# anihcsam/OpenGaussian

Measured on AMD Instinct MI355X. Metric: fwd+bwd Mpix/s at 1080p, 1M Gaussians (RGB+6-D ins_feat); k-means it/s, higher is better.
Workload: dtype f32; 1 GPU; S1M-1080p RGB(SH3)+depth+alpha (all grads) + 6-ch ins_feat (grad to ins_feat) fwd+bwd, ONE fused 9-channel pass; gaussians=1000000, width=1920, height=1080, views_cycled=8, parallelism=single

## Files before the change

opengaussian_amd/csrc/capi.hip:

```cpp
#include <stdarg.h>
#include <stdlib.h>
#include <string.h>

#include <map>
#include <mutex>
#include <string>
#include <vector>

#include "ogs_common.h"

namespace ogs {

static thread_local char g_err[512] = "";

void set_error(const char* fmt, ...) {
    va_list ap;
    va_start(ap, fmt);
    vsnprintf(g_err, sizeof(g_err), fmt, ap);
    va_end(ap);
}

namespace {
struct ProfRec { const char* name; hipEvent_t start, stop; };
int g_prof_mode = 0;
// ... 40 lines not shown
        memset(p, 0, 64);
        g_async_status = static_cast<uint32_t*>(p);
    }
    return g_async_status;
}
int take_async_status() {
    std::lock_guard<std::mutex> lk(g_async_mu);
    if (!g_async_status) return 0;
    return (int)__atomic_exchange_n(g_async_status, 0u, __ATOMIC_ACQ_REL);
}
int check_async_status(const char* where) {
    const int st = take_async_status();
    if (st == 0) return OGS_OK;
    set_error("%s: a kernel of an earlier launch reported status 0x%x%s -- the results of the passes since the last check "
              "are not valid", where, st,
              (st & (int)kAsyncRadixSpin) ? " (one-launch radix pass: a look-back wait exceeded its bound)" : "");
    return OGS_ERR_DEVICE;
}

}
int ogs::blend_prefetch_lines() {
    static const int v = [] {
        const char* e = getenv("OGS_BLEND_PREFETCH");
        const int n = e ? atoi(e) : kPrefetchMax;
        const int lines = (n & 0xFF) > kPrefetchMax ? kPrefetchMax : (n & 0xFF);
#ifdef OGS_EXPERIMENTS
        return n < 0 ? 0 : (lines | (n & 0x300));
#else
        return n < 0 ? 0 : lines;
#endif
    }();
    return v;
}
namespace ogs {

static int bit_length(uint32_t v) {
    int n = 0;
    while (v) { ++n; v >>= 1; }
    return n;
}

static int validate_fwd(const OgsRasterFwdArgs* a, bool images = true) {
    if (!a) { set_error("args == NULL"); return OGS_ERR_INVALID_ARG; }
    if (a->P < 0 || a->W <= 0 || a->H <= 0) { set_error("bad sizes P=%d W=%d H=%d", a->P, a->W, a->H); return OGS_ERR_INVALID_ARG; }
    if (a->C != 3 && a->C != 6 && a->C != 9 && a->C != 12) { set_error("C=%d unsupported (3, 6, 9, 12)", a->C); return OGS_ERR_UNSUPPORTED; }
    if (a->shs == nullptr && a->colors_precomp == nullptr) {
        set_error("provide shs or colors_precomp"); return OGS_ERR_INVALID_ARG;
    }
    if (a->shs != nullptr && (a->colors_precomp != nullptr) != (a->C > 3)) {
        set_error("with shs: C == 3 and no colors_precomp, or C > 3 with colors_precomp holding the C-3 extra channels");
        return OGS_ERR_INVALID_ARG;
    }
    const bool sr = a->scales != nullptr && a->rotations != nullptr;
    if (sr == (a->cov3D_precomp != nullptr) || (a->scales != nullptr) != (a->rotations != nullptr)) {
        set_error("provide exactly one of (scales, rotations) / cov3D_precomp"); return OGS_ERR_INVALID_ARG;
    }
    if (a->shs) {
        if (a->sh_degree < 0 || a->sh_degree > 3 || a->sh_coeffs < (a->sh_degree + 1) * (a->sh_degree + 1)) {
            set_error("sh_degree=%d needs >= %d coefficients, got %d", a->sh_degree, (a->sh_degree + 1) * (a->sh_degree + 1), a->sh_coeffs);
            return OGS_ERR_INVALID_ARG;
        }
    }
    if (!a->bg || !a->viewmatrix || !a->projmatrix || !a->campos || (images && (!a->out_color || !a->out_depth || !a->out_alpha))) {
        set_error("NULL required pointer"); return OGS_ERR_INVALID_ARG;
    }
    if (a->P > 0 && (!a->means3D || !a->opacities || !a->radii || !a->geom_buffer || !a->geom_tmp)) {
        set_error("NULL required per-Gaussian pointer"); return OGS_ERR_INVALID_ARG;
    }
    if (a->num_groups < 0 || (a->num_groups > 1 && a->P > 0 && !a->group_ids)) {
        set_error("num_groups=%d needs group_ids", a->num_groups); return OGS_ERR_INVALID_ARG;
    }
    return OGS_OK;
}

}

using namespace ogs;

extern "C" {

int ogs_version(void) { return 401; }

int ogs_check_async_status(void) { return check_async_status("ogs_check_async_status"); }

int ogs_prof_enable(int on) {
    std::lock_guard<std::mutex> lk(g_prof_mu);
    for (auto& r : g_prof) { g_event_pool.push_back(r.start); g_event_pool.push_back(r.stop); }
    g_prof.clear();
    g_prof_mode = on;
    return OGS_OK;
}

int ogs_prof_filter(const char* prefix) {
    std::lock_guard<std::mutex> lk(g_prof_mu);
    if (!prefix || strlen(prefix) >= sizeof(g_prof_prefix)) { set_error("prof_filter: prefix NULL or longer than %zu", sizeof(g_prof_prefix) - 1); return OGS_ERR_INVALID_ARG; }
    strcpy(g_prof_prefix, prefix);
    return OGS_OK;
}

int ogs_prof_collect(char* buf, size_t n) {
    std::lock_guard<std::mutex> lk(g_prof_mu);
    std::map<std::string, std::pair<long, double>> agg;
    for (auto& r : g_prof) {
        OGS_HIP_CHECK(hipEventSynchronize(r.stop));
        float ms = 0.f;
        OGS_HIP_CHECK(hipEventElapsedTime(&ms, r.start, r.stop));
        auto& a = agg[r.name];
        a.first += 1;
        a.second += ms;
    }
    std::string out = "{";
    bool first = true;
    for (auto& kv : agg) {
        char line[384];
// ... 8 lines not shown
    if (!buf || out.size() + 1 > n) { set_error("prof_collect: buffer too small (%zu needed)", out.size() + 1); return OGS_ERR_SCRATCH_TOO_SMALL; }
    memcpy(buf, out.c_str(), out.size() + 1);
    return OGS_OK;
}
const char* ogs_last_error(void) { return g_err; }

size_t ogs_raster_geom_bytes(int32_t P, int32_t C) { return GeomState::bytes(P > 0 ? P : 1, C); }
size_t ogs_raster_geom_tmp_bytes(int32_t P) { return GeomTmp::bytes(P > 0 ? P : 1); }
size_t ogs_raster_image_bytes(int32_t W, int32_t H) { return ImageState::bytes(W, H); }
size_t ogs_raster_image_bytes_grouped(int32_t W, int32_t H, int32_t G) { return ImageState::bytes(W, H, num_groups_of(G)); }
size_t ogs_raster_binning_tmp_bytes(int64_t D, int32_t, int32_t) { return BinTmp::bytes(D > 0 ? D : 1); }
size_t ogs_raster_sorted_bytes(int64_t D, int32_t C) {
    return align_up((size_t)(D > 0 ? D : 1) * stream_vec4(C) * sizeof(float4));
}
size_t ogs_raster_quad_list_bytes(int64_t D) {
    return align_up((size_t)(5 * (D > 0 ? D : 1) + 2 * kQuadPad) * sizeof(uint32_t));
}
size_t ogs_raster_backward_tmp_bytes(int32_t P) { return align_up((size_t)(P > 0 ? P : 1) * 16 * sizeof(double)); }

int ogs_raster_forward_geometry(const OgsRasterFwdArgs* a, void* stream_, int64_t* num_rendered_host) {
    int rc = validate_fwd(a, false);
    if (rc != OGS_OK) return rc;
    hipStream_t s = static_cast<hipStream_t>(stream_);
    if (num_rendered_host) *num_rendered_host = 0;
    if (a->P == 0) return OGS_OK;
    rc = check_async_status("forward (entry)");
    if (rc != OGS_OK) return rc;
    const GeomState gs = GeomState::carve(a->geom_buffer, a->P, a->C);
    const GeomTmp gt = GeomTmp::carve(a->geom_tmp, a->P);
    if (a->P <= kSmallMaxP) {
        rc = launch_small_geometry(*a, gs, gt, s);
        if (rc != OGS_OK) return rc;
    } else if (per_tile_depth_order(*a)) {
        rc = launch_preprocess(*a, gs, gt, s);
        if (rc != OGS_OK) return rc;
        rc = exclusive_scan_u32(gt.tiles_touched, nullptr, gt.offsets, a->P, gt.num_rendered, gt.sort_tmp, s, a->debug);
        if (rc != OGS_OK) return rc;
    } else {
        rc = launch_preprocess(*a, gs, gt, s);
        if (rc != OGS_OK) return rc;
        const bool sweep = radix_onesweep_enabled(a->P);
        if (sweep) {
            const int shifts[4] = {0, 8, 16, 24}, nbits[4] = {8, 8, 8, 8};
            rc = radix_sort_begin(gt.keys[0], a->P, nullptr, 4, shifts, nbits, gt.sort_tmp, s, a->debug, true);
            if (rc != OGS_OK) return rc;
        }
        for (int pass = 0; pass < 4; ++pass) {
            const int in = pass & 1, out = in ^ 1;
            const bool drop = pass == 0;
            const uint32_t* n_pass = drop ? nullptr : gt.visible();
            rc = sweep ? radix_sort_pass(pass, 4, gt.keys[in], gt.order[in], gt.keys[out], gt.order[out], a->P, 8 * pass, 8, gt.sort_tmp, s, a->debug, n_pass, drop, drop ? gt.visible() : nullptr)
                       : radix_pass(gt.keys[in], gt.order[in], gt.keys[out], gt.order[out], a->P, 8 * pass, 8, gt.sort_tmp, s, a->debug, n_pass, drop, drop ? gt.visible() : nullptr);
            if (rc != OGS_OK) return rc;
        }
        rc = exclusive_scan_u32(gt.tiles_touched, gt.order[0], gt.offsets, a->P, gt.num_rendered, gt.sort_tmp, s, a->debug, gt.visible());
        if (rc != OGS_OK) return rc;
    }
    if (num_rendered_host) {
        uint32_t d = 0;
        OGS_HIP_CHECK(hipMemcpyAsync(&d, gt.num_rendered, sizeof(uint32_t), hipMemcpyDeviceToHost, s));
        OGS_HIP_CHECK(hipStreamSynchronize(s));
        *num_rendered_host = (int64_t)d;
        rc = check_async_status("forward geometry phase");
        if (rc != OGS_OK) return rc;
    }
    return OGS_OK;
}

int ogs_raster_read_num_rendered_async(const OgsRasterFwdArgs* a, void* stream_, uint32_t* host_pinned) {
    if (!a || !host_pinned) { set_error("read_num_rendered_async: NULL pointer"); return OGS_ERR_INVALID_ARG; }
    if (a->P == 0) { *host_pinned = 0; return OGS_OK; }
    const GeomTmp gt = GeomTmp::carve(a->geom_tmp, a->P);
    OGS_HIP_CHECK(hipMemcpyAsync(host_pinned, gt.num_rendered, sizeof(uint32_t), hipMemcpyDeviceToHost,
                                 static_cast<hipStream_t>(stream_)));
    return OGS_OK;
}

static int render_impl(const OgsRasterFwdArgs* a, int64_t D, bool deferred, hipStream_t s,
                       const OgsGroupStatsArgs* stats = nullptr) {
    int rc = validate_fwd(a, stats == nullptr);
    if (rc != OGS_OK) return rc;
    if (!a->image_buffer) { set_error("image_buffer == NULL"); return OGS_ERR_INVALID_ARG; }
    const int G = num_groups_of(a->num_groups);
    const ImageState is = stats ? ImageState::carve_stats(a->image_buffer, a->W, a->H, G)
                                : ImageState::carve(a->image_buffer, a->W, a->H, G);
    const int gx = (a->W + kTile - 1) / kTile, gy = (a->H + kTile - 1) / kTile;
    const int64_t tiles = (int64_t)gx * gy * G;
    if (tiles >= (1ll << 31)) { set_error("%d groups x %d tiles exceed 2^31 virtual tiles", G, gx * gy); return OGS_ERR_UNSUPPORTED; }
    const GeomState gs = GeomState::carve(a->geom_buffer, a->P > 0 ? a->P : 1, a->C);
    const bool per_tile = per_tile_depth_order(*a);
    bool order_ready = false;
    if (D > 0) {
        if (!a->point_list || !a->binning_tmp) { set_error("point_list / binning_tmp == NULL with num_rendered=%lld", (long long)D); return OGS_ERR_INVALID_ARG; }
        if (D >= (1ll << 31)) { set_error("num_rendered=%lld exceeds 2^31", (long long)D); return OGS_ERR_UNSUPPORTED; }
        const GeomTmp gt = GeomTmp::carve(a->geom_tmp, a->P);
        const BinTmp bt = BinTmp::carve(a->binning_tmp, D);
        const int bits = bit_length((uint32_t)(tiles - 1));
        const int passes = bits == 0 ? 1 : (bits + 7) / 8;
        const int per = bits == 0 ? 1 : (bits + passes - 1) / passes;
        uint32_t* vbuf[2];
        vbuf[passes & 1] = a->point_list;
        vbuf[(passes & 1) ^ 1] = bt.vals;
        const uint32_t* n_dev = deferred ? gt.num_rendered : nullptr;
        const bool cull = a->full_binning == 0;
        const bool zero_in_dup = tiles <= (int64_t)a->P;
        rc = launch_duplicate(*a, gs, gt, bt.tile_keys[0], vbuf[0], (uint32_t)D, cull, !per_tile, s,
                              zero_in_dup ? is.ranges : nullptr, zero_in_dup ? (int)tiles : 0);
        if (rc != OGS_OK) return rc;
        const bool sweep = radix_onesweep_enabled(D);
        int shifts[4], nbits[4];
        for (int p = 0; p < passes; ++p) {
            shifts[p] = p * per;
            nbits[p] = (p == passes - 1) ? (bits == 0 ? 1 : bits - shifts[p]) : per;
        }
        if (passes == 2 && (bits & 1)) {
            nbits[0] = bits / 2; shifts[1] = nbits[0]; nbits[1] = bits - nbits[0];
        }
        if (sweep) {
            rc = radix_sort_begin(bt.tile_keys[0], D, n_dev, passes, shifts, nbits, bt.sort_tmp, s, a->debug, cull);
            if (rc != OGS_OK) return rc;
        }
        for (int p = 0; p < passes; ++p) {
            const int in = p & 1, out = in ^ 1;
            const bool drop = cull && p == 0;
            const uint32_t* n_pass = (cull && p > 0) ? bt.kept : n_dev;
            rc = sweep ? radix_sort_pass(p, passes, bt.tile_keys[in], vbuf[in], bt.tile_keys[out], vbuf[out], D, shifts[p], nbits[p], bt.sort_tmp, s, a->debug, n_pass, drop, drop ? bt.kept : nullptr)
                       : radix_pass(bt.tile_keys[in], vbuf[in], bt.tile_keys[out], vbuf[out], D, shifts[p], nbits[p], bt.sort_tmp, s, a->debug, n_pass, drop, drop ? bt.kept : nullptr);
            if (rc != OGS_OK) return rc;
        }
        rc = launch_tile_ranges(bt.tile_keys[passes & 1], D, is.ranges, tiles, s, a->debug, cull ? bt.kept : n_dev, zero_in_dup);
        if (rc != OGS_OK) return rc;
        if (per_tile) {
            const uint32_t* order = launch_tile_order(is, tiles, a->P, s, a->debug);
            order_ready = true;
            rc = launch_tile_depth_sort(is.ranges, tiles, order, a->point_list, gt.keys[0], bt.vals, s, a->debug);
            if (rc != OGS_OK) return rc;
        }
    } else {
        OGS_HIP_CHECK(hipMemsetAsync(is.ranges, 0, (size_t)tiles * sizeof(uint2), s));
    }
    if (stats) return launch_group_stats(*a, *stats, gs, is, s, order_ready);
    if (!a->sorted_rec || !a->quad_list) { set_error("sorted_rec / quad_list == NULL"); return OGS_ERR_INVALID_ARG; }
    return launch_blend_forward(*a, gs, is, D, s, order_ready);
}

int ogs_raster_forward_render(const OgsRasterFwdArgs* a, int64_t D, void* stream_) {
    return render_impl(a, D, false, static_cast<hipStream_t>(stream_));
}

size_t ogs_raster_stats_image_bytes(int32_t W, int32_t H, int32_t G) {
    return ImageState::stats_bytes(W > 0 ? W : 1, H > 0 ? H : 1, num_groups_of(G));
}
size_t ogs_raster_stats_tmp_bytes(int32_t G, int32_t L, int32_t C) {
    return align_up((size_t)num_groups_of(G) * (size_t)((L > 0 ? L : 0) + 1) * (size_t)(C > 0 ? C : 1) * sizeof(int64_t));
}

int ogs_raster_forward_group_stats(const OgsRasterFwdArgs* a, const OgsGroupStatsArgs* st, int64_t D, void* stream_) {
    if (!a || !st) { set_error("forward_group_stats: NULL argument"); return OGS_ERR_INVALID_ARG; }
    if (st->num_labels < 0) { set_error("forward_group_stats: num_labels=%d < 0", st->num_labels); return OGS_ERR_INVALID_ARG; }
    if (!st->labels || !st->max_alpha || !st->count || !st->feat_sum || !st->stats_tmp) {
        set_error("forward_group_stats: NULL labels / output / stats_tmp pointer"); return OGS_ERR_INVALID_ARG;
    }
    if (D < 0) { set_error("forward_group_stats: num_rendered=%lld < 0", (long long)D); return OGS_ERR_INVALID_ARG; }
    if (a->P == 0) D = 0;
    return render_impl(a, D, false, static_cast<hipStream_t>(stream_), st);
}

int ogs_raster_forward_render_deferred(const OgsRasterFwdArgs* a, int64_t capacity, void* stream_) {
    if (capacity <= 0) { set_error("forward_render_deferred: capacity must be > 0"); return OGS_ERR_INVALID_ARG; }
    return render_impl(a, capacity, true, static_cast<hipStream_t>(stream_));
}

int ogs_raster_forward_reblend(const OgsRasterFwdArgs* a, void* stream_) {
// ... 184 lines not shown
```

opengaussian_amd/csrc/ogs_common.h:

```cpp
#pragma once

#include <hip/hip_runtime.h>
#include <stdint.h>
#include <stddef.h>
#include <stdio.h>

#include "../../include/ogs_raster.h"

namespace ogs {

constexpr int kTile = OGS_TILE;
constexpr int kBlock = 256;
constexpr int kWave = 64;
constexpr int kTinyMaxP = 256;
constexpr int kSmallMaxP = 1024;

void set_error(const char* fmt, ...);

#define OGS_HIP_CHECK(expr)                                                              \
    do {                                                                                 \
        hipError_t _e = (expr);                                                          \
        if (_e != hipSuccess) {                                                          \
            ogs::set_error("%s failed: %s (%s:%d)", #expr, hipGetErrorString(_e), __FILE__, __LINE__); \
            return OGS_ERR_HIP;                                                          \
// ... 194 lines not shown
        Carver c(nullptr);
        for (int i = 0; i < 6; ++i) c.take<uint32_t>(P);
        c.take<uint32_t>(64);
        c.take<char>(sort_tmp_bytes(P));
        return c.off;
    }
};

struct BinTmp {
    uint32_t* tile_keys[2];
    uint32_t* vals;
    uint32_t* kept;
    void* sort_tmp;
    static BinTmp carve(void* p, int64_t D) {
        Carver c(p);
        BinTmp b;
        b.tile_keys[0] = c.take<uint32_t>(D);
        b.tile_keys[1] = c.take<uint32_t>(D);
        b.vals = c.take<uint32_t>(D);
        b.kept = c.take<uint32_t>(1);
        b.sort_tmp = c.take<char>(sort_tmp_bytes(D));
        return b;
    }
    static size_t bytes(int64_t D) {
        Carver c(nullptr);
        for (int i = 0; i < 3; ++i) c.take<uint32_t>(D);
        c.take<uint32_t>(1);
        c.take<char>(sort_tmp_bytes(D));
        return c.off;
    }
};

int launch_preprocess(const OgsRasterFwdArgs& a, const GeomState& gs, const GeomTmp& gt, hipStream_t s);
int launch_tiny_geometry(const OgsRasterFwdArgs& a, const GeomState& gs, uint32_t* order, hipStream_t s);
int launch_small_geometry(const OgsRasterFwdArgs& a, const GeomState& gs, const GeomTmp& gt, hipStream_t s);
int launch_tiny_blend(const OgsRasterFwdArgs& a, const GeomState& gs, const uint32_t* order, hipStream_t s);
int launch_reblend(const OgsRasterFwdArgs& a, const ImageState& is, hipStream_t s);
int launch_compact_kept(int W, int H, int C, const ImageState& is_old, const ImageState& is_new, const void* old_rec,
                        const void* old_quad, void* new_rec, void* new_quad, hipStream_t s);
int launch_duplicate(const OgsRasterFwdArgs& a, const GeomState& gs, const GeomTmp& gt, uint32_t* tile_keys,
                     uint32_t* vals, uint32_t capacity, bool drop_unreachable, bool depth_order, hipStream_t s,
                     uint2* zero_ranges = nullptr, int n_zero = 0);
int launch_tile_ranges(const uint32_t* tile_keys_sorted, int64_t D, uint2* ranges, int64_t tiles, hipStream_t s,
                       int debug, const uint32_t* n_dev = nullptr, bool already_zeroed = false);
inline bool per_tile_depth_order(const OgsRasterFwdArgs& a) { return a.num_groups <= 1 && a.P > kSmallMaxP; }
constexpr int kTileSortItems = 16;
constexpr int kTileSortCap = kBlock * kTileSortItems;
constexpr int kWaveSortCap = kTileSortCap / (kBlock / kWave);
int launch_tile_depth_sort(const uint2* ranges, int64_t tiles, const uint32_t* tile_order, uint32_t* point_list,
                           const uint32_t* depth_keys, uint32_t* scratch, hipStream_t s, int debug);
inline int num_groups_of(int g) { return g > 1 ? g : 1; }
int launch_group_stats(const OgsRasterFwdArgs& a, const OgsGroupStatsArgs& st, const GeomState& gs, const ImageState& is,
                       hipStream_t s, bool order_ready = false);
int launch_blend_forward(const OgsRasterFwdArgs& a, const GeomState& gs, const ImageState& is, int64_t D,
                         hipStream_t s, bool order_ready = false);
int launch_blend_backward(const OgsRasterBwdArgs& a, const ImageState& is, void* grad_rec, hipStream_t s);
int launch_preprocess_backward(const OgsRasterBwdArgs& a, const GeomState& gs, const void* grad_rec, hipStream_t s);
inline bool backward_is_features_only(const OgsRasterBwdArgs& a) {
    return a.dL_dcolors != nullptr && a.colors_precomp != nullptr && !a.dL_dmeans2D && !a.dL_dopacity &&
           !a.dL_dmeans3D && !a.dL_dcov3D && !a.dL_dsh && !a.dL_dscales && !a.dL_drotations && !a.dL_dsh_rgb;
}
int launch_sh_grad_from_views(int P, int V, int sh_degree, int sh_coeffs, const float* means3D, const float* campos,
                              const float* dL_drgb, float* dL_dsh, hipStream_t s);
int launch_wave_fold16_test(const float* in, float* out, hipStream_t s);
int launch_tile_order_test(const uint32_t* ranges, int64_t vtiles, uint32_t* order, hipStream_t s);
int launch_mark_visible(int P, const float* means3D, const float* viewmatrix, uint8_t* present, hipStream_t s);
// ... 57 lines not shown
```

opengaussian_amd/csrc/preprocess_fwd.hip:

```cpp
#include "ogs_common.h"

namespace ogs {

namespace {

__constant__ const float kC0 = 0.28209479177387814f;
__constant__ const float kC1 = 0.4886025119029199f;
__constant__ const float kC2[5] = {1.0925484305920792f, -1.0925484305920792f, 0.31539156525252005f,
                                   -1.0925484305920792f, 0.5462742152960396f};
__constant__ const float kC3[7] = {-0.5900435899266435f, 2.890611442640554f, -0.4570457994644658f,
                                   0.3731763325901154f, -0.4570457994644658f, 1.445305721320277f,
                                   -0.5900435899266435f};

struct Cam {
    float V[16];
    float M[16];
    float campos[3];
};

__device__ __forceinline__ void cov3d_from_scale_rot(const float* __restrict__ scales,
                                                     const float* __restrict__ rots, int idx, float mod,
                                                     float cov[6]) {
    const float sx = mod * scales[3 * idx + 0], sy = mod * scales[3 * idx + 1], sz = mod * scales[3 * idx + 2];
    const float4 q = reinterpret_cast<const float4*>(rots)[idx];
// ... 24 lines not shown
    for (int c = 0; c < 3; ++c) res[c] = kC0 * sh[c];
    if (deg > 0) {
#pragma unroll
        for (int c = 0; c < 3; ++c)
            res[c] = res[c] - kC1 * y * sh[3 + c] + kC1 * z * sh[6 + c] - kC1 * x * sh[9 + c];
        if (deg > 1) {
            const float xx = x * x, yy = y * y, zz = z * z, xy = x * y, yz = y * z, xz = x * z;
#pragma unroll
            for (int c = 0; c < 3; ++c)
                res[c] = res[c] + kC2[0] * xy * sh[12 + c] + kC2[1] * yz * sh[15 + c] +
                         kC2[2] * (2.f * zz - xx - yy) * sh[18 + c] + kC2[3] * xz * sh[21 + c] +
                         kC2[4] * (xx - yy) * sh[24 + c];
            if (deg > 2) {
#pragma unroll
                for (int c = 0; c < 3; ++c)
                    res[c] = res[c] + kC3[0] * y * (3.f * xx - yy) * sh[27 + c] + kC3[1] * xy * z * sh[30 + c] +
                             kC3[2] * y * (4.f * zz - xx - yy) * sh[33 + c] +
                             kC3[3] * z * (2.f * zz - 3.f * xx - 3.f * yy) * sh[36 + c] +
                             kC3[4] * x * (4.f * zz - xx - yy) * sh[39 + c] + kC3[5] * z * (xx - yy) * sh[42 + c] +
                             kC3[6] * x * (xx - 3.f * yy) * sh[45 + c];
            }
        }
    }
    clamped = 0;
#pragma unroll
    for (int c = 0; c < 3; ++c) {
        res[c] = res[c] + 0.5f;
        if (res[c] < 0.f) clamped |= 1u << c;
        rgb[c] = fmaxf(res[c], 0.f);
    }
}

template <int C>
__device__ __forceinline__ uint32_t preprocess_one(
    int idx, int W, int H, int sh_degree, int sh_coeffs, float tanfovx, float tanfovy, float focal_x, float focal_y,
    float scale_modifier, const float* __restrict__ means3D, const float* __restrict__ colors_precomp,
    const float* __restrict__ shs, const float* __restrict__ opacities, const float* __restrict__ scales,
    const float* __restrict__ rotations, const float* __restrict__ cov3D_precomp, const float* __restrict__ viewmatrix,
    const float* __restrict__ projmatrix, const float* __restrict__ campos, float4* __restrict__ rec_row,
    uint32_t* __restrict__ clamped_out, int32_t* __restrict__ radii, uint32_t* __restrict__ tiles_touched,
    const int32_t* __restrict__ group_ids, int num_groups) {
    constexpr int NV = rec_vec4(C);
    float V[16], M[16];
#pragma unroll
    for (int i = 0; i < 16; ++i) { V[i] = viewmatrix[i]; M[i] = projmatrix[i]; }

    const float x = means3D[3 * idx + 0], y = means3D[3 * idx + 1], z = means3D[3 * idx + 2];
    const float opacity = opacities[idx];

    float feat[(C + 3) / 4 * 4];
#pragma unroll
    for (int c = 0; c < (C + 3) / 4 * 4; ++c) feat[c] = 0.f;
    uint32_t clamped = 0;

    int radius = 0;
    uint32_t touched = 0;
    float pxl = 0.f, pyl = 0.f, depth = 0.f, cA = 0.f, cB = 0.f, cC = 0.f;

    const float pvx = V[0] * x + V[4] * y + V[8] * z + V[12];
    const float pvy = V[1] * x + V[5] * y + V[9] * z + V[13];
    const float pvz = V[2] * x + V[6] * y + V[10] * z + V[14];
    bool ok = pvz > 0.2f;
    if (group_ids != nullptr) ok = ok && (uint32_t)group_ids[idx] < (uint32_t)num_groups;
    if (ok) {
        const float hx = M[0] * x + M[4] * y + M[8] * z + M[12];
        const float hy = M[1] * x + M[5] * y + M[9] * z + M[13];
        const float hw = M[3] * x + M[7] * y + M[11] * z + M[15];
        const float p_w = 1.0f / (hw + 0.0000001f);
        const float projx = hx * p_w, projy = hy * p_w;
        float cov[6];
        if (cov3D_precomp != nullptr) {
#pragma unroll
            for (int i = 0; i < 6; ++i) cov[i] = cov3D_precomp[6 * idx + i];
        } else {
            cov3d_from_scale_rot(scales, rotations, idx, scale_modifier, cov);
        }
        const float limx = 1.3f * tanfovx, limy = 1.3f * tanfovy;
        const float txtz = pvx / pvz, tytz = pvy / pvz;
        const float tx = fminf(limx, fmaxf(-limx, txtz)) * pvz;
        const float ty = fminf(limy, fmaxf(-limy, tytz)) * pvz;
        const float tz = pvz;
        const float J00 = focal_x / tz;
        const float J02 = -(focal_x * tx) / (tz * tz);
        const float J11 = focal_y / tz;
        const float J12 = -(focal_y * ty) / (tz * tz);
        const float T00 = J00 * V[0] + J02 * V[2];
// ... 17 lines not shown
            const float det_inv = 1.f / det;
            cA = cc * det_inv;
            cB = -cb * det_inv;
            cC = ca * det_inv;
            const float mid = 0.5f * (ca + cc);
            const float sq = sqrtf(fmaxf(0.1f, mid * mid - det));
            const float lam = fmaxf(mid + sq, mid - sq);
            float rad_f = ceilf(3.f * sqrtf(lam));
            if (!(fabsf(rad_f) < 3.0e38f)) rad_f = 0.f;
            const int my_radius = (int)rad_f;
            pxl = ((projx + 1.0f) * (float)W - 1.0f) * 0.5f;
            pyl = ((projy + 1.0f) * (float)H - 1.0f) * 0.5f;
            const int gx = (W + kTile - 1) / kTile, gy = (H + kTile - 1) / kTile;
            const float rf = (float)my_radius;
            auto tr = [](float v) -> int {
                if (!(fabsf(v) < 3.0e38f)) v = 0.f;
                v = fminf(fmaxf(v, -2.0e9f), 2.0e9f);
                return (int)v;
            };
            const int rminx = min(gx, max(0, tr((pxl - rf) / (float)kTile)));
            const int rminy = min(gy, max(0, tr((pyl - rf) / (float)kTile)));
            const int rmaxx = min(gx, max(0, tr((pxl + rf + (float)kTile - 1.0f) / (float)kTile)));
            const int rmaxy = min(gy, max(0, tr((pyl + rf + (float)kTile - 1.0f) / (float)kTile)));
            const int area = (rmaxx - rminx) * (rmaxy - rminy);
            ok = area != 0 && my_radius > 0;
            if (ok) {
                radius = my_radius;
                touched = (uint32_t)area;
                depth = pvz;
            }
        }
    }

    const int coff = shs != nullptr ? 3 : 0;
    if (colors_precomp != nullptr) {
#pragma unroll
        for (int c = 0; c < C; ++c)
            if (c >= coff) feat[c] = colors_precomp[(size_t)idx * (C - coff) + (c - coff)];
    }
    if (shs != nullptr && ok) {
        float rgb[3];
        float cp[3] = {campos[0], campos[1], campos[2]};
        sh_to_rgb(idx, sh_degree, sh_coeffs, shs, x, y, z, cp, rgb, clamped);
        feat[0] = rgb[0]; feat[1] = rgb[1]; feat[2] = rgb[2];
    }

    if (!ok) { pxl = 0.f; pyl = 0.f; cA = cB = cC = 0.f; depth = 0.f; }

    float4* r = rec_row;
    r[0] = make_float4(pxl, pyl, depth, __int_as_float(radius));
    r[1] = make_float4(cA, cB, cC, opacity);
#pragma unroll
    for (int v = 0; v < NV - 2; ++v) r[2 + v] = make_float4(feat[4 * v], feat[4 * v + 1], feat[4 * v + 2], feat[4 * v + 3]);
    clamped_out[idx] = clamped;
    radii[idx] = radius;
    if (tiles_touched) tiles_touched[idx] = touched;
    return ok ? __float_as_uint(depth) : 0xFFFFFFFFu;
}

template <int C>
__global__ __launch_bounds__(kBlock) void preprocess_kernel(
    int P, int W, int H, int sh_degree, int sh_coeffs, float tanfovx, float tanfovy, float focal_x, float focal_y,
    float scale_modifier, const float* __restrict__ means3D, const float* __restrict__ colors_precomp,
    const float* __restrict__ shs, const float* __restrict__ opacities, const float* __restrict__ scales,
    const float* __restrict__ rotations, const float* __restrict__ cov3D_precomp, const float* __restrict__ viewmatrix,
    const float* __restrict__ projmatrix, const float* __restrict__ campos, float4* __restrict__ rec,
    uint32_t* __restrict__ clamped_out, int32_t* __restrict__ radii, uint32_t* __restrict__ tiles_touched,
    uint32_t* __restrict__ depth_keys, uint32_t* __restrict__ order, const int32_t* __restrict__ group_ids,
    int num_groups) {
    constexpr int NV = rec_vec4(C);
    __shared__ float4 s_rec[kBlock * NV];
    const int tid = threadIdx.x;
    const int idx = blockIdx.x * kBlock + tid;
    if (idx < P) {
        depth_keys[idx] = preprocess_one<C>(idx, W, H, sh_degree, sh_coeffs, tanfovx, tanfovy, focal_x, focal_y, scale_modifier,
                                            means3D, colors_precomp, shs, opacities, scales, rotations, cov3D_precomp, viewmatrix,
                                            projmatrix, campos, s_rec + tid * NV, clamped_out, radii, tiles_touched, group_ids,
                                            num_groups);
        if (order) order[idx] = (uint32_t)idx;
    }
    __syncthreads();
    const size_t row0 = (size_t)blockIdx.x * kBlock;
    const int n4 = min(kBlock, P - (int)row0) * NV;
    float4* __restrict__ out = rec + row0 * NV;
    for (int e = tid; e < n4; e += kBlock) out[e] = s_rec[e];
}

template <int C>
__global__ __launch_bounds__(kTinyMaxP) void tiny_geometry_kernel(
    int P, int W, int H, int sh_degree, int sh_coeffs, float tanfovx, float tanfovy, float focal_x, float focal_y,
    float scale_modifier, const float* __restrict__ means3D, const float* __restrict__ colors_precomp,
    const float* __restrict__ shs, const float* __restrict__ opacities, const float* __restrict__ scales,
    const float* __restrict__ rotations, const float* __restrict__ cov3D_precomp, const float* __restrict__ viewmatrix,
    const float* __restrict__ projmatrix, const float* __restrict__ campos, float4* __restrict__ rec,
    uint32_t* __restrict__ clamped_out, int32_t* __restrict__ radii, uint32_t* __restrict__ order) {
    __shared__ uint32_t s_key[kTinyMaxP];
    const int idx = threadIdx.x;
    uint32_t key = 0xFFFFFFFFu;
    if (idx < P)
        key = preprocess_one<C>(idx, W, H, sh_degree, sh_coeffs, tanfovx, tanfovy, focal_x, focal_y, scale_modifier, means3D,
                                colors_precomp, shs, opacities, scales, rotations, cov3D_precomp, viewmatrix, projmatrix,
                                campos, rec + (size_t)idx * rec_vec4(C), clamped_out, radii, nullptr, nullptr, 0);
    s_key[idx] = key;
    __syncthreads();
    if (idx < P) {
        int rank = 0;
        for (int j = 0; j < P; ++j) {
            const uint32_t kj = s_key[j];
            rank += (kj < key || (kj == key && j < idx)) ? 1 : 0;
        }
        order[rank] = (uint32_t)idx;
    }
}

template <int C>
__global__ __launch_bounds__(kSmallMaxP) void small_geometry_kernel(
    int P, int W, int H, int sh_degree, int sh_coeffs, float tanfovx, float tanfovy, float focal_x, float focal_y,
    float scale_modifier, const float* __restrict__ means3D, const float* __restrict__ colors_precomp,
// ... 146 lines not shown
            const bool reach = m >= c.z;
            tile_keys[o] = (drop_unreachable && !reach) ? kDropKey : key;
            vals[o] = g | ((reach ? 1u : 0u) << kReachBit);
        }
    }
}

__global__ __launch_bounds__(kBlock) void mark_visible_kernel(int P, const float* __restrict__ means3D,
                                                              const float* __restrict__ V,
                                                              uint8_t* __restrict__ present) {
    const int idx = blockIdx.x * kBlock + threadIdx.x;
    if (idx >= P) return;
    const float x = means3D[3 * idx], y = means3D[3 * idx + 1], z = means3D[3 * idx + 2];
    const float pvz = V[2] * x + V[6] * y + V[10] * z + V[14];
    present[idx] = pvz > 0.2f ? 1 : 0;
}

template <int C>
int launch_preprocess_c(const OgsRasterFwdArgs& a, const GeomState& gs, const GeomTmp& gt, hipStream_t s) {
    const float focal_x = (float)a.W / (2.0f * a.tanfovx);
    const float focal_y = (float)a.H / (2.0f * a.tanfovy);
    const int grid = (a.P + kBlock - 1) / kBlock;
    static constexpr const char* const kNames[4] = {"preprocess_kernel<3>", "preprocess_kernel<6>", "preprocess_kernel<9>", "preprocess_kernel<12>"};
    OGS_LAUNCH_NAMED(chan_name<C>(kNames), preprocess_kernel<C>, dim3(grid), dim3(kBlock), 0, s, a.P, a.W, a.H, a.sh_degree, a.sh_coeffs,
                       a.tanfovx, a.tanfovy, focal_x, focal_y, a.scale_modifier, a.means3D, a.colors_precomp, a.shs,
                       a.opacities, a.scales, a.rotations, a.cov3D_precomp, a.viewmatrix, a.projmatrix, a.campos,
                       gs.rec, gs.clamped, a.radii, gt.tiles_touched, gt.keys[0],
                       per_tile_depth_order(a) ? (uint32_t*)nullptr : gt.order[0], a.num_groups > 1 ? a.group_ids : (const int32_t*)nullptr, a.num_groups);
    OGS_LAUNCH_CHECK(a.debug, s);
    return OGS_OK;
}

template <int C>
int launch_tiny_geometry_c(const OgsRasterFwdArgs& a, const GeomState& gs, uint32_t* order, hipStream_t s) {
    const float focal_x = (float)a.W / (2.0f * a.tanfovx);
    const float focal_y = (float)a.H / (2.0f * a.tanfovy);
    OGS_LAUNCH(tiny_geometry_kernel<C>, dim3(1), dim3(kTinyMaxP), 0, s, a.P, a.W, a.H, a.sh_degree, a.sh_coeffs, a.tanfovx,
               a.tanfovy, focal_x, focal_y, a.scale_modifier, a.means3D, a.colors_precomp, a.shs, a.opacities, a.scales,
               a.rotations, a.cov3D_precomp, a.viewmatrix, a.projmatrix, a.campos, gs.rec, gs.clamped, a.radii, order);
    OGS_LAUNCH_CHECK(a.debug, s);
    return OGS_OK;
}

template <int C>
int launch_small_geometry_c(const OgsRasterFwdArgs& a, const GeomState& gs, const GeomTmp& gt, hipStream_t s) {
    const float focal_x = (float)a.W / (2.0f * a.tanfovx);
    const float focal_y = (float)a.H / (2.0f * a.tanfovy);
    OGS_LAUNCH(small_geometry_kernel<C>, dim3(1), dim3(kSmallMaxP), 0, s, a.P, a.W, a.H, a.sh_degree, a.sh_coeffs, a.tanfovx,
               a.tanfovy, focal_x, focal_y, a.scale_modifier, a.means3D, a.colors_precomp, a.shs, a.opacities, a.scales,
               a.rotations, a.cov3D_precomp, a.viewmatrix, a.projmatrix, a.campos, gs.rec, gs.clamped, a.radii, gt.order[0],
               gt.offsets, gt.num_rendered, a.num_groups > 1 ? a.group_ids : (const int32_t*)nullptr, a.num_groups);
    OGS_LAUNCH_CHECK(a.debug, s);
    return OGS_OK;
}

}

int launch_small_geometry(const OgsRasterFwdArgs& a, const GeomState& gs, const GeomTmp& gt, hipStream_t s) {
    switch (a.C) {
        case 3: return launch_small_geometry_c<3>(a, gs, gt, s);
        case 6: return launch_small_geometry_c<6>(a, gs, gt, s);
        case 9: return launch_small_geometry_c<9>(a, gs, gt, s);
        case 12: return launch_small_geometry_c<12>(a, gs, gt, s);
        default: set_error("unsupported channel count C=%d (3, 6, 9 or 12)", a.C); return OGS_ERR_UNSUPPORTED;
    }
}

int launch_tiny_geometry(const OgsRasterFwdArgs& a, const GeomState& gs, uint32_t* order, hipStream_t s) {
    switch (a.C) {
        case 3: return launch_tiny_geometry_c<3>(a, gs, order, s);
        case 6: return launch_tiny_geometry_c<6>(a, gs, order, s);
        case 9: return launch_tiny_geometry_c<9>(a, gs, order, s);
        case 12: return launch_tiny_geometry_c<12>(a, gs, order, s);
        default: set_error("unsupported channel count C=%d (3, 6, 9 or 12)", a.C); return OGS_ERR_UNSUPPORTED;
    }
}

int launch_preprocess(const OgsRasterFwdArgs& a, const GeomState& gs, const GeomTmp& gt, hipStream_t s) {
    switch (a.C) {
        case 3: return launch_preprocess_c<3>(a, gs, gt, s);
        case 6: return launch_preprocess_c<6>(a, gs, gt, s);
        case 9: return launch_preprocess_c<9>(a, gs, gt, s);
        case 12: return launch_preprocess_c<12>(a, gs, gt, s);
        default: set_error("unsupported channel count C=%d (3, 6, 9 or 12)", a.C); return OGS_ERR_UNSUPPORTED;
    }
}

int launch_duplicate(const OgsRasterFwdArgs& a, const GeomState& gs, const GeomTmp& gt, uint32_t* tile_keys,
                     uint32_t* vals, uint32_t capacity, bool drop_unreachable, bool depth_order, hipStream_t s, uint2* zero_ranges,
                     int n_zero) {
    if (n_zero > a.P) { set_error("duplicate: %d ranges to clear with %d threads", n_zero, a.P); return OGS_ERR_INVALID_ARG; }
    const int grid = (a.P + kBlock - 1) / kBlock;
    const int32_t* grp = a.num_groups > 1 ? a.group_ids : nullptr;
    if ((a.W + kTile - 1) / kTile > 4095 || (a.H + kTile - 1) / kTile > 4095) {
        set_error("image %dx%d exceeds 4095 tiles per side", a.W, a.H);
        return OGS_ERR_UNSUPPORTED;
    }
    const uint32_t* order = depth_order ? gt.order[0] : nullptr;
    const uint32_t* n_visible = depth_order ? gt.visible() : nullptr;
    switch (rec_vec4(a.C)) {
        case 3: OGS_LAUNCH(duplicate_kernel<3>, dim3(grid), dim3(kBlock), 0, s, a.P, n_visible, a.W, a.H, gs.rec, order, gt.offsets, tile_keys, vals, capacity, grp, drop_unreachable, zero_ranges, n_zero); break;
        case 4: OGS_LAUNCH(duplicate_kernel<4>, dim3(grid), dim3(kBlock), 0, s, a.P, n_visible, a.W, a.H, gs.rec, order, gt.offsets, tile_keys, vals, capacity, grp, drop_unreachable, zero_ranges, n_zero); break;
        case 5: OGS_LAUNCH(duplicate_kernel<5>, dim3(grid), dim3(kBlock), 0, s, a.P, n_visible, a.W, a.H, gs.rec, order, gt.offsets, tile_keys, vals, capacity, grp, drop_unreachable, zero_ranges, n_zero); break;
        default: set_error("unsupported record size"); return OGS_ERR_UNSUPPORTED;
    }
    OGS_LAUNCH_CHECK(a.debug, s);
    return OGS_OK;
}

int launch_mark_visible(int P, const float* means3D, const float* viewmatrix, uint8_t* present, hipStream_t s) {
    const int grid = (P + kBlock - 1) / kBlock;
    OGS_LAUNCH(mark_visible_kernel, dim3(grid), dim3(kBlock), 0, s, P, means3D, viewmatrix, present);
    OGS_LAUNCH_CHECK(0, s);
    return OGS_OK;
}

}
```

Measured before the change: 1453 Mpix/s.

## Split preprocess into geometry and colour kernels, overlap colour with binning on side stream

The forward preprocess kernel is split into a geometry kernel, which computes projection, conic, radii and depth keys, and a colour kernel that evaluates SH and extra channels into the remaining record slots. When P is large, the colour kernel is launched on a low-priority side stream that forks from the main stream and rejoins before blending, so it runs alongside duplication and sorting. SH evaluation is taken off the critical path before the sort, at the cost of an extra launch, a second pass over means3D and radii, and strided partial-record writes.

Measured after the change: 1421 Mpix/s. 2.2% lower.

```diff
diff --git a/opengaussian_amd/csrc/capi.hip b/opengaussian_amd/csrc/capi.hip
--- a/opengaussian_amd/csrc/capi.hip
+++ b/opengaussian_amd/csrc/capi.hip
@@ -96,7 +96,37 @@
     }();
     return v;
 }
+bool ogs::colour_overlap_enabled() {
+    static const bool v = [] { const char* e = getenv("OGS_COLOUR_OVERLAP"); return !(e && atoi(e) == 0); }();
+    return v;
+}
 namespace ogs {
+
+namespace {
+struct SideStream { hipStream_t stream = nullptr; hipEvent_t fork = nullptr, join = nullptr; };
+std::mutex g_side_mu;
+std::map<int, SideStream> g_side;
+int side_stream_locked(SideStream** out) {
+    int dev = 0;
+    OGS_HIP_CHECK(hipGetDevice(&dev));
+    SideStream& ss = g_side[dev];
+    if (!ss.stream) {
+        int least = 0, greatest = 0;
+        OGS_HIP_CHECK(hipDeviceGetStreamPriorityRange(&least, &greatest));
+#ifdef OGS_COLOUR_STREAM_DEFAULT_PRIORITY
+        least = 0;
+#endif
+        hipStream_t st = nullptr;
+        hipEvent_t ef = nullptr, ej = nullptr;
+        OGS_HIP_CHECK(hipStreamCreateWithPriority(&st, hipStreamNonBlocking, least));
+        OGS_HIP_CHECK(hipEventCreateWithFlags(&ef, hipEventDisableTiming));
+        OGS_HIP_CHECK(hipEventCreateWithFlags(&ej, hipEventDisableTiming));
+        ss.stream = st; ss.fork = ef; ss.join = ej;
+    }
+    *out = &ss;
+    return OGS_OK;
+}
+}
 
 static int bit_length(uint32_t v) {
     int n = 0;
@@ -143,7 +173,7 @@
 
 extern "C" {
 
-int ogs_version(void) { return 401; }
+int ogs_version(void) { return 402; }
 
 int ogs_check_async_status(void) { return check_async_status("ogs_check_async_status"); }
 
@@ -218,12 +248,12 @@
         rc = launch_small_geometry(*a, gs, gt, s);
         if (rc != OGS_OK) return rc;
     } else if (per_tile_depth_order(*a)) {
-        rc = launch_preprocess(*a, gs, gt, s);
+        rc = colour_split(*a) ? launch_preprocess_geometry(*a, gs, gt, s) : launch_preprocess(*a, gs, gt, s);
         if (rc != OGS_OK) return rc;
         rc = exclusive_scan_u32(gt.tiles_touched, nullptr, gt.offsets, a->P, gt.num_rendered, gt.sort_tmp, s, a->debug);
         if (rc != OGS_OK) return rc;
     } else {
-        rc = launch_preprocess(*a, gs, gt, s);
+        rc = colour_split(*a) ? launch_preprocess_geometry(*a, gs, gt, s) : launch_preprocess(*a, gs, gt, s);
         if (rc != OGS_OK) return rc;
         const bool sweep = radix_onesweep_enabled(a->P);
         if (sweep) {
@@ -262,20 +292,9 @@
     return OGS_OK;
 }
 
-static int render_impl(const OgsRasterFwdArgs* a, int64_t D, bool deferred, hipStream_t s,
-                       const OgsGroupStatsArgs* stats = nullptr) {
-    int rc = validate_fwd(a, stats == nullptr);
-    if (rc != OGS_OK) return rc;
-    if (!a->image_buffer) { set_error("image_buffer == NULL"); return OGS_ERR_INVALID_ARG; }
-    const int G = num_groups_of(a->num_groups);
-    const ImageState is = stats ? ImageState::carve_stats(a->image_buffer, a->W, a->H, G)
-                                : ImageState::carve(a->image_buffer, a->W, a->H, G);
-    const int gx = (a->W + kTile - 1) / kTile, gy = (a->H + kTile - 1) / kTile;
-    const int64_t tiles = (int64_t)gx * gy * G;
-    if (tiles >= (1ll << 31)) { set_error("%d groups x %d tiles exceed 2^31 virtual tiles", G, gx * gy); return OGS_ERR_UNSUPPORTED; }
-    const GeomState gs = GeomState::carve(a->geom_buffer, a->P > 0 ? a->P : 1, a->C);
-    const bool per_tile = per_tile_depth_order(*a);
-    bool order_ready = false;
+static int render_binning(const OgsRasterFwdArgs* a, int64_t D, bool deferred, hipStream_t s, const GeomState& gs,
+                          const ImageState& is, int64_t tiles, bool per_tile, bool& order_ready) {
+    int rc = OGS_OK;
     if (D > 0) {
         if (!a->point_list || !a->binning_tmp) { set_error("point_list / binning_tmp == NULL with num_rendered=%lld", (long long)D); return OGS_ERR_INVALID_ARG; }
         if (D >= (1ll << 31)) { set_error("num_rendered=%lld exceeds 2^31", (long long)D); return OGS_ERR_UNSUPPORTED; }
@@ -325,6 +344,49 @@
     } else {
         OGS_HIP_CHECK(hipMemsetAsync(is.ranges, 0, (size_t)tiles * sizeof(uint2), s));
     }
+    return OGS_OK;
+}
+
+static int render_impl(const OgsRasterFwdArgs* a, int64_t D, bool deferred, hipStream_t s,
+                       const OgsGroupStatsArgs* stats = nullptr) {
+    int rc = validate_fwd(a, stats == nullptr);
+    if (rc != OGS_OK) return rc;
+    if (!a->image_buffer) { set_error("image_buffer == NULL"); return OGS_ERR_INVALID_ARG; }
+    const int G = num_groups_of(a->num_groups);
+    const ImageState is = stats ? ImageState::carve_stats(a->image_buffer, a->W, a->H, G)
+                                : ImageState::carve(a->image_buffer, a->W, a->H, G);
+    const int gx = (a->W + kTile - 1) / kTile, gy = (a->H + kTile - 1) / kTile;
+    const int64_t tiles = (int64_t)gx * gy * G;
+    if (tiles >= (1ll << 31)) { set_error("%d groups x %d tiles exceed 2^31 virtual tiles", G, gx * gy); return OGS_ERR_UNSUPPORTED; }
+    const GeomState gs = GeomState::carve(a->geom_buffer, a->P > 0 ? a->P : 1, a->C);
+    const bool per_tile = per_tile_depth_order(*a);
+    bool order_ready = false;
+    SideStream* side = nullptr;
+    if (colour_split(*a)) {
+        bool fork = a->debug == 0;
+#ifdef OGS_COLOUR_INSTREAM
+        fork = false;
+#endif
+        if (fork) {
+            hipStreamCaptureStatus cap = hipStreamCaptureStatusNone;
+            OGS_HIP_CHECK(hipStreamIsCapturing(s, &cap));
+            fork = cap == hipStreamCaptureStatusNone;
+        }
+        if (fork) {
+            std::lock_guard<std::mutex> lk(g_side_mu);
+            rc = side_stream_locked(&side);
+            if (rc != OGS_OK) return rc;
+            OGS_HIP_CHECK(hipEventRecord(side->fork, s));
+            OGS_HIP_CHECK(hipStreamWaitEvent(side->stream, side->fork, 0));
+            rc = launch_preprocess_colour(*a, gs, side->stream);
+            OGS_HIP_CHECK(hipEventRecord(side->join, side->stream));
+        } else {
+            rc = launch_preprocess_colour(*a, gs, s);
+        }
+    }
+    if (rc == OGS_OK) rc = render_binning(a, D, deferred, s, gs, is, tiles, per_tile, order_ready);
+    if (side) OGS_HIP_CHECK(hipStreamWaitEvent(s, side->join, 0));
+    if (rc != OGS_OK) return rc;
     if (stats) return launch_group_stats(*a, *stats, gs, is, s, order_ready);
     if (!a->sorted_rec || !a->quad_list) { set_error("sorted_rec / quad_list == NULL"); return OGS_ERR_INVALID_ARG; }
     return launch_blend_forward(*a, gs, is, D, s, order_ready);
diff --git a/opengaussian_amd/csrc/ogs_common.h b/opengaussian_amd/csrc/ogs_common.h
--- a/opengaussian_amd/csrc/ogs_common.h
+++ b/opengaussian_amd/csrc/ogs_common.h
@@ -250,6 +250,16 @@
 };
 
 int launch_preprocess(const OgsRasterFwdArgs& a, const GeomState& gs, const GeomTmp& gt, hipStream_t s);
+int launch_preprocess_geometry(const OgsRasterFwdArgs& a, const GeomState& gs, const GeomTmp& gt, hipStream_t s);
+int launch_preprocess_colour(const OgsRasterFwdArgs& a, const GeomState& gs, hipStream_t s);
+#ifndef OGS_COLOUR_OVERLAP_MIN_P
+#define OGS_COLOUR_OVERLAP_MIN_P 300000
+#endif
+constexpr int kColourOverlapMinP = OGS_COLOUR_OVERLAP_MIN_P;
+bool colour_overlap_enabled();
+inline bool colour_split(const OgsRasterFwdArgs& a) {
+    return a.P > kSmallMaxP && a.P >= kColourOverlapMinP && colour_overlap_enabled();
+}
 int launch_tiny_geometry(const OgsRasterFwdArgs& a, const GeomState& gs, uint32_t* order, hipStream_t s);
 int launch_small_geometry(const OgsRasterFwdArgs& a, const GeomState& gs, const GeomTmp& gt, hipStream_t s);
 int launch_tiny_blend(const OgsRasterFwdArgs& a, const GeomState& gs, const uint32_t* order, hipStream_t s);
diff --git a/opengaussian_amd/csrc/preprocess_fwd.hip b/opengaussian_amd/csrc/preprocess_fwd.hip
--- a/opengaussian_amd/csrc/preprocess_fwd.hip
+++ b/opengaussian_amd/csrc/preprocess_fwd.hip
@@ -80,26 +80,19 @@
 }
 
 template <int C>
-__device__ __forceinline__ uint32_t preprocess_one(
-    int idx, int W, int H, int sh_degree, int sh_coeffs, float tanfovx, float tanfovy, float focal_x, float focal_y,
-    float scale_modifier, const float* __restrict__ means3D, const float* __restrict__ colors_precomp,
-    const float* __restrict__ shs, const float* __restrict__ opacities, const float* __restrict__ scales,
-    const float* __restrict__ rotations, const float* __restrict__ cov3D_precomp, const float* __restrict__ viewmatrix,
-    const float* __restrict__ projmatrix, const float* __restrict__ campos, float4* __restrict__ rec_row,
-    uint32_t* __restrict__ clamped_out, int32_t* __restrict__ radii, uint32_t* __restrict__ tiles_touched,
-    const int32_t* __restrict__ group_ids, int num_groups) {
-    constexpr int NV = rec_vec4(C);
+__device__ __forceinline__ uint32_t preprocess_geometry_one(
+    int idx, int W, int H, float tanfovx, float tanfovy, float focal_x, float focal_y,
+    float scale_modifier, const float* __restrict__ means3D, const float* __restrict__ opacities,
+    const float* __restrict__ scales, const float* __restrict__ rotations, const float* __restrict__ cov3D_precomp,
+    const float* __restrict__ viewmatrix, const float* __restrict__ projmatrix, float4* __restrict__ rec_row,
+    int32_t* __restrict__ radii, uint32_t* __restrict__ tiles_touched, const int32_t* __restrict__ group_ids,
+    int num_groups, bool& ok_out) {
     float V[16], M[16];
 #pragma unroll
     for (int i = 0; i < 16; ++i) { V[i] = viewmatrix[i]; M[i] = projmatrix[i]; }
 
     const float x = means3D[3 * idx + 0], y = means3D[3 * idx + 1], z = means3D[3 * idx + 2];
     const float opacity = opacities[idx];
-
-    float feat[(C + 3) / 4 * 4];
-#pragma unroll
-    for (int c = 0; c < (C + 3) / 4 * 4; ++c) feat[c] = 0.f;
-    uint32_t clamped = 0;
 
     int radius = 0;
     uint32_t touched = 0;
@@ -183,6 +176,29 @@
         }
     }
 
+    if (!ok) { pxl = 0.f; pyl = 0.f; cA = cB = cC = 0.f; depth = 0.f; }
+
+    float4* r = rec_row;
+    r[0] = make_float4(pxl, pyl, depth, __int_as_float(radius));
+    r[1] = make_float4(cA, cB, cC, opacity);
+    radii[idx] = radius;
+    if (tiles_touched) tiles_touched[idx] = touched;
+    ok_out = ok;
+    return ok ? __float_as_uint(depth) : 0xFFFFFFFFu;
+}
+
+template <int C>
+__device__ __forceinline__ void preprocess_colour_one(int idx, bool ok, int sh_degree, int sh_coeffs,
+                                                      const float* __restrict__ means3D,
+                                                      const float* __restrict__ colors_precomp,
+                                                      const float* __restrict__ shs, const float* __restrict__ campos,
+                                                      float4* __restrict__ feat_row, uint32_t* __restrict__ clamped_out) {
+    constexpr int NV = rec_vec4(C);
+    float feat[(C + 3) / 4 * 4];
+#pragma unroll
+    for (int c = 0; c < (C + 3) / 4 * 4; ++c) feat[c] = 0.f;
+    uint32_t clamped = 0;
+
     const int coff = shs != nullptr ? 3 : 0;
     if (colors_precomp != nullptr) {
 #pragma unroll
@@ -192,21 +208,31 @@
     if (shs != nullptr && ok) {
         float rgb[3];
         float cp[3] = {campos[0], campos[1], campos[2]};
+        const float x = means3D[3 * idx + 0], y = means3D[3 * idx + 1], z = means3D[3 * idx + 2];
         sh_to_rgb(idx, sh_degree, sh_coeffs, shs, x, y, z, cp, rgb, clamped);
         feat[0] = rgb[0]; feat[1] = rgb[1]; feat[2] = rgb[2];
     }
 
-    if (!ok) { pxl = 0.f; pyl = 0.f; cA = cB = cC = 0.f; depth = 0.f; }
-
-    float4* r = rec_row;
-    r[0] = make_float4(pxl, pyl, depth, __int_as_float(radius));
-    r[1] = make_float4(cA, cB, cC, opacity);
-#pragma unroll
-    for (int v = 0; v < NV - 2; ++v) r[2 + v] = make_float4(feat[4 * v], feat[4 * v + 1], feat[4 * v + 2], feat[4 * v + 3]);
+#pragma unroll
+    for (int v = 0; v < NV - 2; ++v) feat_row[v] = make_float4(feat[4 * v], feat[4 * v + 1], feat[4 * v + 2], feat[4 * v + 3]);
     clamped_out[idx] = clamped;
-    radii[idx] = radius;
-    if (tiles_touched) tiles_touched[idx] = touched;
-    return ok ? __float_as_uint(depth) : 0xFFFFFFFFu;
+}
+
+template <int C>
+__device__ __forceinline__ uint32_t preprocess_one(
+    int idx, int W, int H, int sh_degree, int sh_coeffs, float tanfovx, float tanfovy, float focal_x, float focal_y,
+    float scale_modifier, const float* __restrict__ means3D, const float* __restrict__ colors_precomp,
+    const float* __restrict__ shs, const float* __restrict__ opacities, const float* __restrict__ scales,
+    const float* __restrict__ rotations, const float* __restrict__ cov3D_precomp, const float* __restrict__ viewmatrix,
+    const float* __restrict__ projmatrix, const float* __restrict__ campos, float4* __restrict__ rec_row,
+    uint32_t* __restrict__ clamped_out, int32_t* __restrict__ radii, uint32_t* __restrict__ tiles_touched,
+    const int32_t* __restrict__ group_ids, int num_groups) {
+    bool ok;
+    const uint32_t key = preprocess_geometry_one<C>(idx, W, H, tanfovx, tanfovy, focal_x, focal_y, scale_modifier, means3D,
+                                                    opacities, scales, rotations, cov3D_precomp, viewmatrix, projmatrix,
+                                                    rec_row, radii, tiles_touched, group_ids, num_groups, ok);
+    preprocess_colour_one<C>(idx, ok, sh_degree, sh_coeffs, means3D, colors_precomp, shs, campos, rec_row + 2, clamped_out);
+    return key;
 }
 
 template <int C>
@@ -235,6 +261,64 @@
     const int n4 = min(kBlock, P - (int)row0) * NV;
     float4* __restrict__ out = rec + row0 * NV;
     for (int e = tid; e < n4; e += kBlock) out[e] = s_rec[e];
+}
+
+template <int C>
+__global__ __launch_bounds__(kBlock) void preprocess_geometry_kernel(
+    int P, int W, int H, float tanfovx, float tanfovy, float focal_x, float focal_y, float scale_modifier,
+    const float* __restrict__ means3D, const float* __restrict__ opacities, const float* __restrict__ scales,
+    const float* __restrict__ rotations, const float* __restrict__ cov3D_precomp, const float* __restrict__ viewmatrix,
+    const float* __restrict__ projmatrix, float4* __restrict__ rec, int32_t* __restrict__ radii,
+    uint32_t* __restrict__ tiles_touched, uint32_t* __restrict__ depth_keys, uint32_t* __restrict__ order,
+    const int32_t* __restrict__ group_ids, int num_groups) {
+    constexpr int NV = rec_vec4(C);
+    __shared__ float4 s_rec[kBlock * 2];
+    const int tid = threadIdx.x;
+    const int idx = blockIdx.x * kBlock + tid;
+    if (idx < P) {
+        bool ok;
+        depth_keys[idx] = preprocess_geometry_one<C>(idx, W, H, tanfovx, tanfovy, focal_x, focal_y, scale_modifier, means3D,
+                                                     opacities, scales, rotations, cov3D_precomp, viewmatrix, projmatrix,
+                                                     s_rec + tid * 2, radii, tiles_touched, group_ids, num_groups, ok);
+        if (order) order[idx] = (uint32_t)idx;
+    }
+    __syncthreads();
+    const size_t row0 = (size_t)blockIdx.x * kBlock;
+    const int n4 = min(kBlock, P - (int)row0) * 2;
+    float4* __restrict__ out = rec + row0 * NV;
+    for (int e = tid; e < n4; e += kBlock) out[(size_t)(e >> 1) * NV + (e & 1)] = s_rec[e];
+}
+
+template <int C>
+__global__ __launch_bounds__(kBlock) void preprocess_colour_kernel(
+    int P, int sh_degree, int sh_coeffs, const float* __restrict__ means3D, const float* __restrict__ colors_precomp,
+    const float* __restrict__ shs, const float* __restrict__ campos, const int32_t* __restrict__ radii,
+    float4* __restrict__ rec, uint32_t* __restrict__ clamped_out) {
+    constexpr int NV = rec_vec4(C), NF = NV - 2;
+    __shared__ float4 s_feat[kBlock * NF];
+    const int tid = threadIdx.x;
+#ifdef OGS_COLOUR_GRID_CAP
+    for (int blk = blockIdx.x; blk * kBlock < P; blk += gridDim.x) {
+#else
+    {
+        const int blk = blockIdx.x;
+#endif
+        const int idx = blk * kBlock + tid;
+        if (idx < P)
+            preprocess_colour_one<C>(idx, radii[idx] > 0, sh_degree, sh_coeffs, means3D, colors_precomp, shs, campos,
+                                     s_feat + tid * NF, clamped_out);
+        __syncthreads();
+        const size_t row0 = (size_t)blk * kBlock;
+        const int n4 = min(kBlock, P - (int)row0) * NF;
+        float4* __restrict__ out = rec + row0 * NV + 2;
+        for (int e = tid; e < n4; e += kBlock) {
+            const int row = e / NF;
+            out[(size_t)row * NV + (e - row * NF)] = s_feat[e];
+        }
+#ifdef OGS_COLOUR_GRID_CAP
+        __syncthreads();
+#endif
+    }
 }
 
 template <int C>
@@ -447,6 +531,36 @@
 }
 
 template <int C>
+int launch_preprocess_geometry_c(const OgsRasterFwdArgs& a, const GeomState& gs, const GeomTmp& gt, hipStream_t s) {
+    const float focal_x = (float)a.W / (2.0f * a.tanfovx);
+    const float focal_y = (float)a.H / (2.0f * a.tanfovy);
+    const int grid = (a.P + kBlock - 1) / kBlock;
+    static constexpr const char* const kNames[4] = {"preprocess_geometry_kernel<3>", "preprocess_geometry_kernel<6>",
+                                                    "preprocess_geometry_kernel<9>", "preprocess_geometry_kernel<12>"};
+    OGS_LAUNCH_NAMED(chan_name<C>(kNames), preprocess_geometry_kernel<C>, dim3(grid), dim3(kBlock), 0, s, a.P, a.W, a.H, a.tanfovx,
+                     a.tanfovy, focal_x, focal_y, a.scale_modifier, a.means3D, a.opacities, a.scales, a.rotations,
+                     a.cov3D_precomp, a.viewmatrix, a.projmatrix, gs.rec, a.radii, gt.tiles_touched, gt.keys[0],
+                     per_tile_depth_order(a) ? (uint32_t*)nullptr : gt.order[0],
+                     a.num_groups > 1 ? a.group_ids : (const int32_t*)nullptr, a.num_groups);
+    OGS_LAUNCH_CHECK(a.debug, s);
+    return OGS_OK;
+}
+
+template <int C>
+int launch_preprocess_colour_c(const OgsRasterFwdArgs& a, const GeomState& gs, hipStream_t s) {
+    int grid = (a.P + kBlock - 1) / kBlock;
+#ifdef OGS_COLOUR_GRID_CAP
+    grid = grid < OGS_COLOUR_GRID_CAP ? grid : OGS_COLOUR_GRID_CAP;
+#endif
+    static constexpr const char* const kNames[4] = {"preprocess_colour_kernel<3>", "preprocess_colour_kernel<6>",
+                                                    "preprocess_colour_kernel<9>", "preprocess_colour_kernel<12>"};
+    OGS_LAUNCH_NAMED(chan_name<C>(kNames), preprocess_colour_kernel<C>, dim3(grid), dim3(kBlock), 0, s, a.P, a.sh_degree,
+                     a.sh_coeffs, a.means3D, a.colors_precomp, a.shs, a.campos, a.radii, gs.rec, gs.clamped);
+    OGS_LAUNCH_CHECK(a.debug, s);
+    return OGS_OK;
+}
+
+template <int C>
 int launch_tiny_geometry_c(const OgsRasterFwdArgs& a, const GeomState& gs, uint32_t* order, hipStream_t s) {
     const float focal_x = (float)a.W / (2.0f * a.tanfovx);
     const float focal_y = (float)a.H / (2.0f * a.tanfovy);
@@ -501,6 +615,26 @@
     }
 }
 
+int launch_preprocess_geometry(const OgsRasterFwdArgs& a, const GeomState& gs, const GeomTmp& gt, hipStream_t s) {
+    switch (a.C) {
+        case 3: return launch_preprocess_geometry_c<3>(a, gs, gt, s);
+        case 6: return launch_preprocess_geometry_c<6>(a, gs, gt, s);
+        case 9: return launch_preprocess_geometry_c<9>(a, gs, gt, s);
+        case 12: return launch_preprocess_geometry_c<12>(a, gs, gt, s);
+        default: set_error("unsupported channel count C=%d (3, 6, 9 or 12)", a.C); return OGS_ERR_UNSUPPORTED;
+    }
+}
+
+int launch_preprocess_colour(const OgsRasterFwdArgs& a, const GeomState& gs, hipStream_t s) {
+    switch (a.C) {
+        case 3: return launch_preprocess_colour_c<3>(a, gs, s);
+        case 6: return launch_preprocess_colour_c<6>(a, gs, s);
+        case 9: return launch_preprocess_colour_c<9>(a, gs, s);
+        case 12: return launch_preprocess_colour_c<12>(a, gs, s);
+        default: set_error("unsupported channel count C=%d (3, 6, 9 or 12)", a.C); return OGS_ERR_UNSUPPORTED;
+    }
+}
+
 int launch_duplicate(const OgsRasterFwdArgs& a, const GeomState& gs, const GeomTmp& gt, uint32_t* tile_keys,
                      uint32_t* vals, uint32_t capacity, bool drop_unreachable, bool depth_order, hipStream_t s, uint2* zero_ranges,
                      int n_zero) {
```
